# Borx25/CPU-Raytracing-experiments

Hardware: AMD Instinct MI355X
Metric: Mray/s (primary+bounce) (higher is better)
Workload: dtype f32; 1 GPU; cfg4: 4096x4096 px, S(100000) spheres + SAH BVH, MIS, Policy.max_bounces=9 (primary+8 bounces), 5 buckets, 64 accumulations/step; fixed image, tile rows split over the GPUs; image=4096x4096, spheres=100000, max_bounces=9, buckets=5, parallelism=single GPU, batches_in_flight=1, accumulations_per_batch=63, accumulations_per_batch_limit=63

## Files before the change

cpu-raytracing-experiments_amd/csrc/mirt_capi.hip:

```cpp
#include "../../include/mirt.h"
#include "kernels.hpp"
#include "bvh_layout.hpp"
#include "bvh_build.hpp"
#include "lbvh_build.hpp"

#include <hip/hip_runtime.h>
#include <algorithm>
#include <cstdarg>
#include <cstdio>
#include <cstdlib>
#include <cstring>
#include <string>
#include <vector>

using namespace mirt;

namespace {

thread_local std::string g_create_error;

struct DeviceBuffer {
	void* ptr = nullptr;
	size_t bytes = 0;
	hipError_t ensure(size_t want) {
		if (want <= bytes && ptr) return hipSuccess;
		if (ptr) { (void)hipFree(ptr); ptr = nullptr; bytes = 0; }
		if (want == 0) return hipSuccess;
		hipError_t e = hipMalloc(&ptr, want);
		if (e == hipSuccess) bytes = want;
		return e;
	}
	void release() { if (ptr) (void)hipFree(ptr); ptr = nullptr; bytes = 0; }
	template <class T> T* as() const { return static_cast<T*>(ptr); }
};

struct ScopedBuffer : DeviceBuffer {
	ScopedBuffer() = default;
	ScopedBuffer(const ScopedBuffer&) = delete;
	ScopedBuffer& operator=(const ScopedBuffer&) = delete;
	~ScopedBuffer() { release(); }
};

struct TimedLaunch { int klass; hipEvent_t start, stop; };

struct PipeSlot {
	hipStream_t stream = nullptr;
	DeviceBuffer arena;
	DeviceBuffer counts;
	DeviceBuffer contrib;
	DeviceBuffer fat;
	DeviceBuffer cand;
	hipEvent_t batch_done = nullptr;
	hipEvent_t merged = nullptr;
	hipEvent_t aov_done = nullptr;
	bool in_use = false;
	StreamBuf stream_buf[2]{};
	ShadowBuf shadow_buf{};
	HitRec* hit = nullptr;
};

}

struct mirt_ctx {
	int device = 0;
	int n_cu = 256;
	hipStream_t stream = nullptr;
	std::string error;

	mirt_policy policy{ 16, 5, 1, 0, 0, 0, 0, 0, 0, 0, 0, 0 };
	uint32_t width = 0, height = 0, h_tiles = 0, v_tiles = 0;
	uint32_t first_tile = 0, n_tiles = 0;
	uint32_t run_tiles = 0, stride_tiles = 0;
	uint32_t accumulations = 0;
	bool have_scene = false, have_camera = false;

	DeviceBuffer recs, recs_wide, spheres, prim_mat, light_sphere, light_emit, mat_albedo, mat_emission, mat_ggx, hdri;
	SceneDev scene{};
	std::vector<float> gloss_decay;
	uint32_t stream_order = 0;
	DeviceBuffer gloss_decay_dev;
	bool gloss_decay_dev_valid = false;
	CameraParams camera{};
	uint32_t bvh_depth = 0;
	bool allow_half = true;

	DeviceBuffer accumulator;
	uint32_t aov_on = 0;
	DeviceBuffer aov;
	hipEvent_t aov_prev = nullptr;
	DeviceBuffer framebuffer;
	float* frame_host = nullptr;
	size_t frame_host_bytes = 0;
	DeviceBuffer counters;
	std::vector<PipeSlot> slots;
	uint64_t planned_for = 0;
	uint32_t batch_mem_cap = 256;
	uint32_t capacity = 0;
	uint32_t seg_cap = 0;
	uint32_t arena_bounces = 0;
	uint64_t batch_seq = 0;

	uint32_t deferred = 0;
	uint32_t tune_trace_wgs = 2, tune_shade_wgs = 3, tune_chunk = kChunkMax, tune_leaf_batch = kLeafBatch, tune_refill_idle = kRefillIdle, tune_wide = 1;
	bool debug_poison_contrib = false;
	std::vector<TimedLaunch> pending;
	std::vector<hipEvent_t> free_events;
	mirt_kernel_times times{};
};

namespace {

int fail(mirt_ctx* ctx, int code, const char* fmt, ...) {
	char buf[512];
	va_list ap; va_start(ap, fmt); vsnprintf(buf, sizeof buf, fmt, ap); va_end(ap);
	if (ctx) ctx->error = buf; else g_create_error = buf;
	return code;
}
#define HIP_TRY(ctx, expr) do { hipError_t _e = (expr); if (_e != hipSuccess) return fail(ctx, MIRT_ERR_HIP, "%s: %s", #expr, hipGetErrorString(_e)); } while (0)

constexpr uint32_t kMaxBatch = 256;
constexpr uint64_t kBatchRays = 1024ull << 20;
constexpr uint64_t kSerialRays = 96ull << 20;
constexpr size_t kStreamPlanes = 2 * 10 + 2 + 14;
uint32_t pix_bits_of(const mirt_ctx* c) { uint32_t b = 8; while ((1ull << b) < static_cast<uint64_t>(c->n_tiles) * kTileSize) b++; return b; }
uint32_t max_slots(const mirt_ctx* c) {
	const uint64_t n_pix = std::max<uint64_t>(static_cast<uint64_t>(c->n_tiles) * kTileSize, 1);
	const uint64_t by_slots = ((1ull << 30) - 3ull * kSegs * kShadeBlock) / n_pix;
	return static_cast<uint32_t>(std::max<uint64_t>(std::min<uint64_t>(std::min<uint64_t>(kMaxBatch, 1u << (30u - std::min<uint32_t>(pix_bits_of(c), 24u))), by_slots), 1));
}
uint32_t batch_floor(const mirt_ctx* c) { return std::max<uint32_t>(std::min<uint32_t>(c->policy.buckets, 5u), 1u); }
uint32_t batch_limit(const mirt_ctx* c) {
	if (c->policy.max_batch) return std::min(c->policy.max_batch, max_slots(c));
	const uint64_t n_pix = static_cast<uint64_t>(c->n_tiles) * kTileSize;
	if (n_pix == 0) return 1;
	const uint64_t b = std::max<uint64_t>((kBatchRays + n_pix / 2) / n_pix, batch_floor(c));
	return static_cast<uint32_t>(std::min<uint64_t>(std::min<uint64_t>(b, max_slots(c)), std::max<uint32_t>(c->batch_mem_cap, 1u)));
// ... 6 lines not shown
	if (blocks < 1) blocks = 1;
	return static_cast<uint32_t>(blocks);
}

constexpr uint32_t kLdsPerCu = 160u * 1024u;
struct LdsPlan {
	uint32_t stack16;
	uint32_t rec_bytes, lds_recs, lds_spheres, staged_bytes, stack_bytes;
	uint32_t launch_bytes;
	uint32_t wgs_per_cu;
};
LdsPlan lds_plan(const mirt_ctx* c) {
	const SceneDev& s = c->scene;
	const bool half = s.half_boxes != 0;
	LdsPlan p{};
	p.stack16 = (half && s.n_recs <= 32768 && s.n_spheres <= 32768) ? 1u : 0u;
	p.rec_bytes = (half && !s.wide) ? 32u : 64u;
	p.stack_bytes = half ? (p.stack16 ? kLdsStack * kTraceBlock * 2u : kLdsStackWide * kTraceBlock * 4u) : kLdsStack * kTraceBlock * 4u;
	const uint32_t budget = half ? (p.stack16 ? 48u * 1024u : 32u * 1024u) : 96u * 1024u;
	if (static_cast<uint64_t>(s.n_recs) * p.rec_bytes + static_cast<uint64_t>(s.n_spheres) * 16u <= budget) { p.lds_recs = s.n_recs; p.lds_spheres = s.n_spheres; }
	else { p.lds_recs = std::min<uint32_t>(s.n_recs, budget / p.rec_bytes); p.lds_spheres = 0; }
	p.staged_bytes = p.lds_recs * p.rec_bytes + p.lds_spheres * 16u;
	p.launch_bytes = c->policy.use_bvh ? p.staged_bytes + p.stack_bytes : kBruteChunk * 16u;
	p.wgs_per_cu = std::min(std::max(kLdsPerCu / p.launch_bytes, 1u), c->tune_trace_wgs);
	return p;
}
uint32_t trace_lds(const mirt_ctx* c) { return lds_plan(c).launch_bytes; }
uint32_t trace_grid(const mirt_ctx* c, uint64_t work_items) {
	uint64_t blocks = (work_items + kTraceBlock - 1) / kTraceBlock;
	const uint64_t cap = static_cast<uint64_t>(c->n_cu) * lds_plan(c).wgs_per_cu;
	if (blocks > cap) blocks = cap;
	if (blocks < 1) blocks = 1;
	return static_cast<uint32_t>(blocks);
}

hipError_t sync_all(mirt_ctx* c) {
	for (PipeSlot& sl : c->slots) if (sl.stream) { hipError_t e = hipStreamSynchronize(sl.stream); if (e != hipSuccess) return e; }
	return hipStreamSynchronize(c->stream);
}
constexpr uint32_t kQueueWords = kSegs * kSegPitch;
constexpr uint32_t kFatCapacity = 1u << 16;
struct BatchCounters {
	uint32_t* w; uint32_t nb, seg_cap;
	static size_t words(uint32_t nb) { return static_cast<size_t>(2 * nb + 2) * kQueueWords + static_cast<size_t>(nb) * 4 + 8; }
	Queue queue(uint32_t k) const { return Queue{ w + static_cast<size_t>(k) * kQueueWords, seg_cap }; }
	uint32_t* word(uint32_t k) const { return w + static_cast<size_t>(2 * nb + 2) * kQueueWords + k; }
	Queue stream_queue(uint32_t b) const { return queue(b); }
	Queue shadow_queue(uint32_t b) const { return queue(nb + 1 + b); }
	Queue empty_queue() const { return queue(2 * nb + 1); }
	uint32_t* closest_work(uint32_t b) const { return word(b); }
	uint32_t* shadow_work(uint32_t b) const { return word(nb + b); }
	FatList fat_closest(uint32_t b, uint32_t* lists) const { return FatList{ word(2 * nb + b), lists, kFatCapacity }; }
	FatList fat_shadow(uint32_t b, uint32_t* lists) const { return FatList{ word(3 * nb + b), lists + kFatCapacity, kFatCapacity }; }
	uint32_t* cand_work() const { return word(4 * nb); }
	uint32_t* unused_fat_count() const { return word(4 * nb + 1); }
	uint32_t* listed_pixels() const { return word(4 * nb + 2); }
};
BatchCounters batch_counters(const mirt_ctx* c, const PipeSlot& sl) { return BatchCounters{ sl.counts.as<uint32_t>(), c->policy.max_bounces, c->seg_cap }; }
uint32_t wanted_slots(const mirt_ctx* c) {
	if (c->policy.streams) return std::min<uint32_t>(c->policy.streams, 8u);
	return static_cast<uint64_t>(c->n_tiles) * kTileSize * batch_limit(c) >= kSerialRays ? 1u : 3u;
}
uint64_t streams_bytes(const mirt_ctx* c) {
	const uint64_t rays = static_cast<uint64_t>(c->n_tiles) * kTileSize * batch_limit(c);
	return wanted_slots(c) * (rays * 4u * kStreamPlanes + rays * 12u);
}

void plan_batches(mirt_ctx* c) {
	const uint64_t n_pix = static_cast<uint64_t>(c->n_tiles) * kTileSize;
	if (c->policy.max_batch || n_pix == 0 || c->planned_for == n_pix) return;
	c->batch_mem_cap = kMaxBatch;
	size_t free_b = 0, total_b = 0, own = 0;
	for (const PipeSlot& sl : c->slots) own += sl.arena.bytes + sl.contrib.bytes;
	if (hipSetDevice(c->device) == hipSuccess && hipMemGetInfo(&free_b, &total_b) == hipSuccess)
		while (batch_limit(c) > batch_floor(c) && streams_bytes(c) > (free_b + own) / 5 * 4) c->batch_mem_cap = std::max(batch_limit(c) / 2, batch_floor(c));
	c->planned_for = n_pix;
}

int ensure_streams(mirt_ctx* c) {
	const uint64_t n_pix = static_cast<uint64_t>(c->n_tiles) * kTileSize;
	if (n_pix * batch_limit(c) == 0) return MIRT_OK;
	plan_batches(c);
	const uint64_t cap64 = n_pix * batch_limit(c);
	if (n_pix > (1u << 24)) return fail(c, MIRT_ERR_ARG, "more than 2^24 pixels per context (%llu); shard the tile range", (unsigned long long)n_pix);
	if (cap64 + 3ull * kSegs * kShadeBlock > (1ull << 30)) return fail(c, MIRT_ERR_ARG, "stream capacity %llu too large", (unsigned long long)cap64);
	const uint32_t seg_cap = static_cast<uint32_t>((((cap64 + kShadeBlock - 1) / kShadeBlock + kSegs - 1) / kSegs + 2) * kShadeBlock);
	const uint32_t cap = seg_cap * kSegs;
	const uint32_t nb = c->policy.max_bounces;
	const uint32_t want = wanted_slots(c);
	const size_t acc_bytes = static_cast<size_t>(c->n_tiles) * batch_limit(c) * 3 * kTileSize * sizeof(float);
	if (cap == c->capacity && nb == c->arena_bounces && c->slots.size() == want && c->slots[0].contrib.bytes >= acc_bytes) return MIRT_OK;
	HIP_TRY(c, sync_all(c));
	c->aov_prev = nullptr;
	while (c->slots.size() > want) {
		PipeSlot& sl = c->slots.back();
		sl.arena.release(); sl.counts.release(); sl.contrib.release(); sl.fat.release(); sl.cand.release();
		if (sl.batch_done) (void)hipEventDestroy(sl.batch_done);
		if (sl.merged) (void)hipEventDestroy(sl.merged);
		if (sl.aov_done) (void)hipEventDestroy(sl.aov_done);
		if (sl.stream) (void)hipStreamDestroy(sl.stream);
		c->slots.pop_back();
	}
	while (c->slots.size() < want) {
		PipeSlot sl;
		HIP_TRY(c, hipStreamCreateWithFlags(&sl.stream, hipStreamNonBlocking));
		HIP_TRY(c, hipEventCreateWithFlags(&sl.batch_done, hipEventDisableTiming));
		HIP_TRY(c, hipEventCreateWithFlags(&sl.merged, hipEventDisableTiming));
		c->slots.push_back(sl);
	}
	const size_t planes = kStreamPlanes;
	const size_t plane_bytes = (static_cast<size_t>(cap) * 4 + 255) & ~static_cast<size_t>(255);
	for (PipeSlot& sl : c->slots) {
		sl.in_use = false;
		hipError_t e = sl.arena.ensure(planes * plane_bytes);
		const char* what = "ray streams";
		if (e == hipSuccess) { e = sl.counts.ensure(BatchCounters::words(nb) * sizeof(uint32_t)); what = "queue counters"; }
		if (e == hipSuccess) { e = sl.fat.ensure(2u * kFatCapacity * sizeof(uint32_t)); what = "fat-ray lists"; }
		if (e == hipSuccess) { e = sl.cand.ensure(static_cast<size_t>(n_pix) * kCandStride * sizeof(uint32_t)); what = "candidate lists"; }
		if (e == hipSuccess) { e = sl.contrib.ensure(acc_bytes); what = "contribution buffer"; }
		if (e != hipSuccess) {
			(void)hipGetLastError();
			if (e == hipErrorOutOfMemory && !c->policy.max_batch && batch_limit(c) > batch_floor(c)) {
				for (PipeSlot& other : c->slots) { other.arena.release(); other.contrib.release(); }
				c->capacity = 0;
				c->batch_mem_cap = std::max(batch_limit(c) / 2, batch_floor(c));
				return ensure_streams(c);
			}
			return fail(c, MIRT_ERR_HIP, "%s (%zu bytes of ray streams per batch in flight): %s", what, planes * plane_bytes, hipGetErrorString(e));
		}
		char* p = sl.arena.as<char>();
		auto take = [&]() { void* r = p; p += plane_bytes; return r; };
		for (int b = 0; b < 2; b++) {
			StreamBuf& s = sl.stream_buf[b];
			s.px = (float*)take(); s.py = (float*)take(); s.pz = (float*)take();
			s.dx = (float*)take(); s.dy = (float*)take(); s.dz = (float*)take();
			s.tr = (float*)take(); s.tg = (float*)take(); s.tb = (float*)take();
			s.path = (uint32_t*)take();
		}
		sl.hit = (HitRec*)take(); (void)take();
		ShadowBuf& h = sl.shadow_buf;
		h.px = (float*)take(); h.py = (float*)take(); h.pz = (float*)take();
		h.dx = (float*)take(); h.dy = (float*)take(); h.dz = (float*)take(); h.tfar = (float*)take();
		h.sr = (float*)take(); h.sg = (float*)take(); h.sb = (float*)take();
		h.er = (float*)take(); h.eg = (float*)take(); h.eb = (float*)take();
		h.dest = (uint32_t*)take();
	}
	c->capacity = cap;
	c->seg_cap = seg_cap;
	c->arena_bounces = nb;
	return MIRT_OK;
}

size_t aov_floats(const mirt_ctx* c) { return c->aov_on ? static_cast<size_t>(c->n_tiles) * kAovPlanes * kTileSize : 0; }
int alloc_aov(mirt_ctx* c) {
	const size_t floats = aov_floats(c);
	HIP_TRY(c, c->aov.ensure(floats * sizeof(float)));
	if (floats) HIP_TRY(c, hipMemsetAsync(c->aov.ptr, 0, floats * sizeof(float), c->stream));
	return MIRT_OK;
}

int alloc_accumulator(mirt_ctx* c) {
	const size_t floats = static_cast<size_t>(c->n_tiles) * c->policy.buckets * 3 * kTileSize;
	HIP_TRY(c, sync_all(c));
	HIP_TRY(c, c->accumulator.ensure(floats * sizeof(float)));
	if (floats) HIP_TRY(c, hipMemsetAsync(c->accumulator.ptr, 0, floats * sizeof(float), c->stream));
	if (c->aov_on) { const int r = alloc_aov(c); if (r) return r; }
	HIP_TRY(c, hipMemsetAsync(c->counters.ptr, 0, sizeof(DevCounters), c->stream));
	HIP_TRY(c, hipStreamSynchronize(c->stream));
	for (PipeSlot& sl : c->slots) sl.in_use = false;
	c->accumulations = 0;
	return MIRT_OK;
// ... 47 lines not shown
	fp.inv_h_tiles = fp.h_tiles ? 1.0f / static_cast<float>(fp.h_tiles) : 0.0f;
	fp.inv_run_tiles = 1.0f / static_cast<float>(fp.run_tiles);
	return fp;
}

SceneDev trace_scene(const mirt_ctx* c) {
	SceneDev sc = c->scene;
	sc.use_bvh = c->policy.use_bvh;
	sc.chunk_max = c->tune_chunk; sc.leaf_batch = c->tune_leaf_batch; sc.refill_idle = c->tune_refill_idle;
	return sc;
}

const decltype(&k_trace<true, kPrimaryNone>) kTrace[2][3] = {
	{ k_trace<true, kPrimaryNone>, k_trace<true, kPrimaryAll>, k_trace<true, kPrimaryList> },
	{ k_trace<false, kPrimaryNone>, k_trace<false, kPrimaryAll>, k_trace<false, kPrimaryList> } };
const decltype(&k_trace_fat<true, kPrimaryNone>) kTraceFat[2][3] = {
	{ k_trace_fat<true, kPrimaryNone>, k_trace_fat<true, kPrimaryAll>, k_trace_fat<true, kPrimaryList> },
	{ k_trace_fat<false, kPrimaryNone>, k_trace_fat<false, kPrimaryAll>, k_trace_fat<false, kPrimaryList> } };
const decltype(&k_primary_cand<true>) kPrimaryCand[2] = { k_primary_cand<true>, k_primary_cand<false> };
const decltype(&k_primary_hits<true>) kPrimaryHits[2] = { k_primary_hits<true>, k_primary_hits<false> };
const decltype(&k_shade<false, false>) kShade[2][2] = { { k_shade<false, false>, k_shade<false, true> }, { k_shade<true, false>, k_shade<true, true> } };
const decltype(&k_tile_stream<false>) kTileStream[2] = { k_tile_stream<false>, k_tile_stream<true> };
static_assert(kPrimaryNone == 0 && kPrimaryAll == 1 && kPrimaryList == 2, "kTrace / kTraceFat are indexed by PRIMARY");

struct TraceLaunch {
	StreamBuf in; HitRec* hit;
	Queue closest_queue; uint32_t* closest_work;
	ShadowBuf sh; ShadowSink sink;
	Queue shadow_queue; uint32_t* shadow_work;
	FatList fat_closest, fat_shadow;
	const uint32_t* listed_pixels;
	DevCounters* ctr;
};
void launch_trace(const mirt_ctx* c, hipStream_t st, const SceneDev& sc, const FrameParams& fp, uint64_t n_rays, bool count, int primary, const TraceLaunch& t) {
	hipLaunchKernelGGL(kTrace[!count][primary], dim3(trace_grid(c, n_rays)), dim3(kTraceBlock), trace_lds(c), st, sc, fp, t.in, t.hit, t.closest_queue, t.closest_work,
	                   t.sh, t.sink, t.shadow_queue, t.shadow_work, t.fat_closest, t.fat_shadow, t.ctr);
	const uint32_t fat_grid = sc.n_spheres > 4096 ? static_cast<uint32_t>(c->n_cu) * 2u : 64u;
	if (sc.use_bvh) hipLaunchKernelGGL(kTraceFat[!count][primary], dim3(fat_grid), dim3(1024), 0, st, sc, fp, t.in, t.hit, t.fat_closest, t.sh, t.sink, t.fat_shadow, t.ctr, t.listed_pixels);
}

int launch_tile_stream(mirt_ctx* c, hipStream_t st, const SceneDev& sc, const FrameParams& fp, uint32_t batch_n, float* contrib, DevCounters* ctr, bool count) {
	if (!c->gloss_decay_dev_valid) {
		HIP_TRY(c, sync_all(c));
		HIP_TRY(c, c->gloss_decay_dev.ensure(std::max<size_t>(c->gloss_decay.size(), 1) * sizeof(float)));
		if (!c->gloss_decay.empty()) HIP_TRY(c, hipMemcpy(c->gloss_decay_dev.ptr, c->gloss_decay.data(), c->gloss_decay.size() * sizeof(float), hipMemcpyHostToDevice));
		c->gloss_decay_dev_valid = true;
	}
	Bracket t(c, MIRT_K_TRACE, st);
	hipLaunchKernelGGL(kTileStream[c->policy.brdf != 0], dim3(c->n_tiles * batch_n), dim3(kTileSize), 0, st, sc, fp, contrib, ctr, c->mat_ggx.as<float4>(),
	                   c->gloss_decay_dev.as<float>(), static_cast<uint32_t>(c->gloss_decay.size()), count ? 1u : 0u);
	return MIRT_OK;
}

int launch_first_hit_aov(mirt_ctx* c, PipeSlot& sl, hipStream_t st, const SceneDev& sc, const FrameParams& fp) {
	const bool pipelined = c->slots.size() > 1;
	if (pipelined) {
		if (!sl.aov_done) HIP_TRY(c, hipEventCreateWithFlags(&sl.aov_done, hipEventDisableTiming));
		if (c->aov_prev && c->aov_prev != sl.aov_done) HIP_TRY(c, hipStreamWaitEvent(st, c->aov_prev, 0));
	}
	{ Bracket t(c, MIRT_K_RESOLVE, st);
	  const uint32_t grid = static_cast<uint32_t>(std::min<uint64_t>((static_cast<uint64_t>(fp.n_pix) + kBlock - 1) / kBlock, static_cast<uint64_t>(c->n_cu) * 64u));
	  hipLaunchKernelGGL(k_first_hit_aov, dim3(grid), dim3(kBlock), 0, st, sc, fp, sl.hit, c->policy.brdf ? c->mat_ggx.as<float4>() : c->scene.mat_albedo, c->aov.as<float>()); }
	if (pipelined) { HIP_TRY(c, hipEventRecord(sl.aov_done, st)); c->aov_prev = sl.aov_done; }
	return MIRT_OK;
}

int launch_batch(mirt_ctx* c, uint32_t batch_n) {
	FrameParams fp = frame_params(c, c->accumulations, batch_n);
	const uint32_t nb = c->policy.max_bounces;
	const uint64_t total = static_cast<uint64_t>(fp.n_pix) * batch_n;
	if (total == 0) { c->accumulations += batch_n; return MIRT_OK; }
	const bool pipelined = c->slots.size() > 1;
	PipeSlot& sl = c->slots[c->batch_seq % c->slots.size()];
	hipStream_t st = pipelined ? sl.stream : c->stream;
	const BatchCounters bc = batch_counters(c, sl);
	const float qn = c->camera.orient[0] * c->camera.orient[0] + c->camera.orient[1] * c->camera.orient[1] + c->camera.orient[2] * c->camera.orient[2] + c->camera.orient[3] * c->camera.orient[3];
	const bool bundle = c->policy.use_bvh && c->scene.n_recs != 0 && !c->policy.trace_primary_rays && batch_n >= 3 && c->camera.z != 0.0f && std::fabs(qn - 1.0f) < 1e-4f;
	DevCounters* ctr = c->counters.as<DevCounters>();
	const float4* mat_ggx = c->mat_ggx.as<float4>();
	float* contrib = sl.contrib.as<float>();
	uint32_t* fat_lists = sl.fat.as<uint32_t>();
	const SceneDev sc = trace_scene(c);
	const bool count = c->policy.count_traffic != 0;
	const uint32_t sgrid = static_cast<uint32_t>(std::min<uint64_t>((total + kShadeBlock - 1) / kShadeBlock, static_cast<uint64_t>(c->n_cu) * c->tune_shade_wgs));
	{
		const uint64_t n_chunks = (static_cast<uint64_t>(fp.n_pix) + kShadeBlock - 1) / kShadeBlock;
		const uint64_t want = (8ull * sgrid + n_chunks - 1) / n_chunks;
		fp.first_groups = static_cast<uint32_t>(std::min<uint64_t>(std::max<uint64_t>(want, 1), batch_n));
	}

	if (pipelined && sl.in_use) HIP_TRY(c, hipStreamWaitEvent(st, sl.merged, 0));
	if (c->debug_poison_contrib)
		HIP_TRY(c, hipMemsetD32Async(reinterpret_cast<hipDeviceptr_t>(sl.contrib.ptr), 0x7fc0deadu, sl.contrib.bytes / sizeof(float), st));
	HIP_TRY(c, hipMemsetAsync(bc.w, 0, BatchCounters::words(nb) * sizeof(uint32_t), st));
	if (c->stream_order) {
		const int r = launch_tile_stream(c, st, sc, fp, batch_n, contrib, ctr, count);
		if (r) return r;
	} else {
		for (uint32_t bounce = 0; bounce < nb; bounce++) {
			const StreamBuf& in = sl.stream_buf[bounce & 1u];
			const StreamBuf& out = sl.stream_buf[(bounce & 1u) ^ 1u];
			const bool shadow_pending = fp.mis && bounce > 0;
			const bool lists = bounce == 0 && bundle;
			{ Bracket t(c, MIRT_K_TRACE, st);
			  if (lists) {
			    const FatList none{ bc.unused_fat_count(), fat_lists, 0u };
			    hipLaunchKernelGGL(kPrimaryCand[!count], dim3(trace_grid(c, fp.n_pix)), dim3(kTraceBlock), trace_lds(c), st, sc, fp, sl.cand.as<uint32_t>(), bundle_half_angle(c),
			                       bc.cand_work(), none, ctr, in.path, bc.listed_pixels());
			    const uint32_t hgrid = static_cast<uint32_t>(std::min<uint64_t>((static_cast<uint64_t>(fp.n_pix) + kBlock - 1) / kBlock, static_cast<uint64_t>(c->n_cu) * 64u));
			    hipLaunchKernelGGL(kPrimaryHits[!count], dim3(hgrid), dim3(kBlock), 0, st, sc, fp, sl.cand.as<uint32_t>(), sl.hit, ctr);
			  }
			  const ShadowSink sink{ in.path, in.px, in.py, in.pz, contrib, batch_n, fp.pix_bits, nullptr };
			  const TraceLaunch tl{ in, sl.hit, lists ? Queue{ bc.listed_pixels(), 0u } : bc.stream_queue(bounce), bc.closest_work(bounce),
			                        sl.shadow_buf, sink, shadow_pending ? bc.shadow_queue(bounce - 1) : bc.empty_queue(), bc.shadow_work(shadow_pending ? bounce - 1 : 0),
			                        bc.fat_closest(bounce, fat_lists), bc.fat_shadow(bounce, fat_lists), bc.listed_pixels(), ctr };
			  launch_trace(c, st, sc, fp, total, count, lists ? kPrimaryList : bounce == 0 ? kPrimaryAll : kPrimaryNone, tl); }
			if (bounce == 0 && c->aov_on) { const int r = launch_first_hit_aov(c, sl, st, sc, fp); if (r) return r; }
			{ Bracket t(c, MIRT_K_SHADE, st);
			  const float decay = bounce < c->gloss_decay.size() ? c->gloss_decay[bounce] : 0.0f;
			  hipLaunchKernelGGL(kShade[bounce == 0][c->policy.brdf != 0], dim3(sgrid), dim3(kShadeBlock), 0, st, sc, fp, in, sl.hit, out, sl.shadow_buf, bounce,
			                     bc.stream_queue(bounce), bc.stream_queue(bounce + 1), bc.shadow_queue(bounce), contrib, ctr, mat_ggx, decay); }
		}
	}
	HIP_TRY(c, hipGetLastError());
	if (pipelined) {
		HIP_TRY(c, hipEventRecord(sl.batch_done, st));
		HIP_TRY(c, hipStreamWaitEvent(c->stream, sl.batch_done, 0));
	}
	{ Bracket t(c, MIRT_K_RESOLVE);
	  hipLaunchKernelGGL(k_merge_contrib, dim3(grid_for(c, static_cast<uint64_t>(c->n_tiles) * (kTileSize / 4u))), dim3(kBlock), 0, c->stream,
	                     c->accumulator.as<float4>(), sl.contrib.as<float4>(), c->n_tiles, c->policy.buckets, batch_n, fp.acc_base); }
	HIP_TRY(c, hipGetLastError());
	if (pipelined) { HIP_TRY(c, hipEventRecord(sl.merged, c->stream)); sl.in_use = true; }
	c->batch_seq++;
	c->accumulations += batch_n;
	if (c->policy.profile && c->pending.size() > 512) harvest(c);
	return MIRT_OK;
}

template <class T>
int upload(mirt_ctx* c, DeviceBuffer& buf, const std::vector<T>& host) {
	HIP_TRY(c, buf.ensure(std::max<size_t>(host.size(), 1) * sizeof(T)));
	if (!host.empty()) HIP_TRY(c, hipMemcpyAsync(buf.ptr, host.data(), host.size() * sizeof(T), hipMemcpyHostToDevice, c->stream));
	return MIRT_OK;
}

int check_ready(mirt_ctx* c) {
	if (!c) return MIRT_ERR_ARG;
	if (!c->have_scene) return fail(c, MIRT_ERR_STATE, "mirt_set_scene has not been called");
	if (!c->have_camera) return fail(c, MIRT_ERR_STATE, "mirt_set_camera has not been called");
	if (c->width == 0 && c->height == 0) return fail(c, MIRT_ERR_STATE, "mirt_resize has not been called");
	return MIRT_OK;
}

int flush_deferred(mirt_ctx* c) {
	if (!c->deferred) return MIRT_OK;
	const uint32_t n = c->deferred;
	c->deferred = 0;
	HIP_TRY(c, hipSetDevice(c->device));
	int r = ensure_streams(c); if (r) return r;
	return launch_batch(c, n);
}

struct SceneArgs {
	const mirt_sphere *geometry, *bvh_prims; uint32_t n_spheres;
	const mirt_bvh_node* nodes; uint32_t n_nodes;
	const mirt_material* materials; uint32_t n_materials;
	const int32_t* lights; uint32_t n_lights;
// ... 156 lines not shown
	tl.closest_queue = bc.stream_queue(0); tl.closest_work = bc.closest_work(0);
	tl.shadow_queue = bc.shadow_queue(0); tl.shadow_work = bc.shadow_work(0);
	tl.fat_closest = bc.fat_closest(0, fat.as<uint32_t>()); tl.fat_shadow = bc.fat_shadow(0, fat.as<uint32_t>());
	tl.ctr = ctr.as<DevCounters>();
	{ Bracket t(c, MIRT_K_TRACE);
	  launch_trace(c, c->stream, trace_scene(c), FrameParams{}, n, false, kPrimaryNone, tl); }
	hipError_t e = hipGetLastError();
	if (e == hipSuccess) e = hipStreamSynchronize(c->stream);
	if (e == hipSuccess) e = hipMemcpy(result, res.ptr, result_bytes, hipMemcpyDeviceToHost);
	if (e != hipSuccess) return fail(c, MIRT_ERR_HIP, "%s: %s", who, hipGetErrorString(e));
	return MIRT_OK;
}

}

extern "C" {

const char* mirt_last_error(const mirt_ctx* ctx) { return ctx ? ctx->error.c_str() : g_create_error.c_str(); }

int mirt_create(int device, mirt_ctx** out) {
	if (!out) return fail(nullptr, MIRT_ERR_ARG, "out is NULL");
	*out = nullptr;
	int n = 0;
	hipError_t e = hipGetDeviceCount(&n);
	if (e != hipSuccess || n <= 0) return fail(nullptr, MIRT_ERR_NO_DEVICE, "no HIP device available (%s); mirt has no CPU path", hipGetErrorString(e));
	if (device < 0 || device >= n) return fail(nullptr, MIRT_ERR_ARG, "device %d out of range (have %d)", device, n);
	e = hipSetDevice(device);
	if (e != hipSuccess) return fail(nullptr, MIRT_ERR_HIP, "hipSetDevice: %s", hipGetErrorString(e));
	mirt_ctx* c = new mirt_ctx();
	c->device = device;
	if (const char* e = std::getenv("MIRT_TUNE_CHUNK")) c->tune_chunk = static_cast<uint32_t>(std::min(std::max(std::atoi(e), 64), 65536)) & ~63u;
	if (const char* e = std::getenv("MIRT_TUNE_REFILL_IDLE")) c->tune_refill_idle = static_cast<uint32_t>(std::min(std::max(std::atoi(e), 1), 64));
	if (const char* e = std::getenv("MIRT_TUNE_WIDE")) c->tune_wide = std::atoi(e) != 0 ? 1u : 0u;
	if (const char* e = std::getenv("MIRT_TUNE_LEAF_BATCH")) c->tune_leaf_batch = static_cast<uint32_t>(std::min(std::max(std::atoi(e), 1), 64));
	if (const char* e = std::getenv("MIRT_TUNE_TRACE_WGS")) c->tune_trace_wgs = std::atoi(e) == 1 ? 1u : 2u;
	if (const char* e = std::getenv("MIRT_TUNE_SHADE_WGS")) c->tune_shade_wgs = static_cast<uint32_t>(std::min(std::max(std::atoi(e), 1), 16));
	if (const char* e = std::getenv("MIRT_DEBUG_POISON_CONTRIB")) c->debug_poison_contrib = std::atoi(e) != 0;
	hipDeviceProp_t prop;
	if (hipGetDeviceProperties(&prop, device) == hipSuccess) c->n_cu = prop.multiProcessorCount > 0 ? prop.multiProcessorCount : 256;
	e = hipStreamCreateWithFlags(&c->stream, hipStreamNonBlocking);
	if (e == hipSuccess) e = c->counters.ensure(sizeof(DevCounters));
	if (e == hipSuccess) e = hipMemsetAsync(c->counters.ptr, 0, sizeof(DevCounters), c->stream);
	if (e != hipSuccess) { int r = fail(nullptr, MIRT_ERR_HIP, "context setup: %s", hipGetErrorString(e)); delete c; return r; }
	*out = c;
	return MIRT_OK;
}

int mirt_destroy(mirt_ctx* c) {
	if (!c) return MIRT_ERR_ARG;
	(void)hipSetDevice(c->device);
	(void)sync_all(c);
	harvest(c);
	for (PipeSlot& sl : c->slots) {
		sl.arena.release(); sl.counts.release(); sl.contrib.release(); sl.fat.release(); sl.cand.release();
		if (sl.batch_done) (void)hipEventDestroy(sl.batch_done);
		if (sl.merged) (void)hipEventDestroy(sl.merged);
		if (sl.aov_done) (void)hipEventDestroy(sl.aov_done);
		if (sl.stream) (void)hipStreamDestroy(sl.stream);
	}
	c->slots.clear();
	for (hipEvent_t e : c->free_events) (void)hipEventDestroy(e);
	DeviceBuffer* bufs[] = { &c->recs, &c->recs_wide, &c->spheres, &c->prim_mat, &c->light_sphere, &c->light_emit, &c->mat_albedo, &c->mat_emission,
	                         &c->mat_ggx, &c->hdri, &c->accumulator, &c->aov, &c->framebuffer, &c->counters, &c->gloss_decay_dev };
	for (DeviceBuffer* b : bufs) b->release();
	if (c->frame_host) (void)hipHostFree(c->frame_host);
	if (c->stream) (void)hipStreamDestroy(c->stream);
	delete c;
	return MIRT_OK;
}

int mirt_set_scene(mirt_ctx* c, const mirt_sphere* geometry, const mirt_sphere* bvh_prims, uint32_t n_spheres,
                   const mirt_bvh_node* nodes, uint32_t n_nodes, const mirt_material* materials, uint32_t n_materials,
                   const int32_t* lights, uint32_t n_lights, const float ambient_color[3],
                   const float* hdri_rgba, uint32_t hdri_w, uint32_t hdri_h) {
	if (!c) return MIRT_ERR_ARG;
	{ const int fr = flush_deferred(c); if (fr) return fr; }
	const SceneArgs a{ geometry, bvh_prims, n_spheres, nodes, n_nodes, materials, n_materials, lights, n_lights, ambient_color, hdri_rgba, hdri_w, hdri_h };
	int r = check_scene_args(c, a); if (r) return r;
	HIP_TRY(c, hipSetDevice(c->device));
	const SceneTables t = flatten_tables(a);
	SceneRecords tree;
	if ((r = upload(c, c->spheres, t.sph)) || (r = build_scene_records(c, a, t.sph, tree)) || (r = upload(c, c->prim_mat, t.pm)) ||
	    (r = upload(c, c->light_sphere, t.lsp)) || (r = upload(c, c->light_emit, t.lem)) || (r = upload(c, c->mat_albedo, t.alb)) ||
	    (r = upload(c, c->mat_emission, t.emi)) || (r = upload(c, c->mat_ggx, t.ggx)) || (r = upload(c, c->hdri, t.sky))) return r;
	HIP_TRY(c, hipStreamSynchronize(c->stream));
	commit_scene(c, a, tree);
	if ((r = plan_trace_lds(c))) return r;
	c->have_scene = true;
	return MIRT_OK;
}

int mirt_set_camera(mirt_ctx* c, const float pos[3], const float orient_xyzw[4], float half_width, float half_height, float z, float exposure) {
	if (!c) return MIRT_ERR_ARG;
	if (!pos || !orient_xyzw) return fail(c, MIRT_ERR_ARG, "pos / orient is NULL");
	if (c->have_camera && std::memcmp(c->camera.pos, pos, 12) == 0 && std::memcmp(c->camera.orient, orient_xyzw, 16) == 0 &&
	    c->camera.half_width == half_width && c->camera.half_height == half_height && c->camera.z == z && c->camera.exposure == exposure)
		return MIRT_OK;
	{ const int fr = flush_deferred(c); if (fr) return fr; }
	for (int k = 0; k < 3; k++) c->camera.pos[k] = pos[k];
	for (int k = 0; k < 4; k++) c->camera.orient[k] = orient_xyzw[k];
	c->camera.half_width = half_width; c->camera.half_height = half_height; c->camera.z = z; c->camera.exposure = exposure;
	c->have_camera = true;
	return MIRT_OK;
}

int mirt_set_policy(mirt_ctx* c, const mirt_policy* p) {
	if (!c || !p) return MIRT_ERR_ARG;
	if (p->max_bounces < 1 || p->max_bounces > 1024) return fail(c, MIRT_ERR_ARG, "max_bounces %u out of range", p->max_bounces);
	if (p->buckets < 1 || p->buckets > MIRT_MAX_BUCKETS) return fail(c, MIRT_ERR_ARG, "buckets %u out of range 1..%u", p->buckets, MIRT_MAX_BUCKETS);
	if (p->brdf > 1) return fail(c, MIRT_ERR_ARG, "brdf %u is neither 0 (Lambertian) nor 1 (GGX)", p->brdf);
	{ const int fr = flush_deferred(c); if (fr) return fr; }
	HIP_TRY(c, hipSetDevice(c->device));
	HIP_TRY(c, sync_all(c));
	const bool realloc_acc = p->buckets != c->policy.buckets;
	const bool replan = p->max_batch != c->policy.max_batch || p->streams != c->policy.streams || p->buckets != c->policy.buckets || p->max_bounces != c->policy.max_bounces;
	c->policy = *p;
	if (replan) c->planned_for = 0;
	if (realloc_acc && c->n_tiles) { int r = alloc_accumulator(c); if (r) return r; }
	return MIRT_OK;
}
int mirt_set_gloss_decay(mirt_ctx* c, const float* decay, uint32_t n) {
	if (!c) return MIRT_ERR_ARG;
	if (!decay) n = 0;
	if (n > 1024) return fail(c, MIRT_ERR_ARG, "gloss decay table of %u entries (at most 1024, the max_bounces limit)", n);
	for (uint32_t i = 0; i < n; i++)
		if (!(decay[i] >= 0.0f && decay[i] <= 1.0f)) return fail(c, MIRT_ERR_ARG, "gloss decay[%u] = %g is not in [0, 1]", i, static_cast<double>(decay[i]));
	{ const int fr = flush_deferred(c); if (fr) return fr; }
	c->gloss_decay.assign(decay, decay + n);
	c->gloss_decay_dev_valid = false;
	return MIRT_OK;
}
int mirt_set_stream_order(mirt_ctx* c, uint32_t exact) {
	if (!c) return MIRT_ERR_ARG;
	if (exact > 1) return fail(c, MIRT_ERR_ARG, "stream order %u is neither 0 (any order, FMA form for every ray) nor 1 (the reference's slots and scalar tail)", exact);
	if (exact == c->stream_order) return MIRT_OK;
	if (exact && c->aov_on) return fail(c, MIRT_ERR_STATE, "exact stream order keeps no hit records (k_tile_stream runs a tile's whole bounce loop in one launch), so it cannot feed the first-hit AOVs: call mirt_set_aov(ctx, 0) first");
	{ const int fr = flush_deferred(c); if (fr) return fr; }
	c->stream_order = exact;
	return MIRT_OK;
}
int mirt_get_stream_order(const mirt_ctx* c, uint32_t* exact) { if (!c || !exact) return MIRT_ERR_ARG; *exact = c->stream_order; return MIRT_OK; }
int mirt_get_policy(const mirt_ctx* c, mirt_policy* p) {
	if (!c || !p) return MIRT_ERR_ARG;
	*p = c->policy;
	plan_batches(const_cast<mirt_ctx*>(c));
	p->max_batch = batch_limit(c);
	p->streams = wanted_slots(c);
	return MIRT_OK;
}

int mirt_resize(mirt_ctx* c, uint32_t width, uint32_t height) {
	if (!c) return MIRT_ERR_ARG;
	if (width > 65536 || height > 65536) return fail(c, MIRT_ERR_ARG, "size %ux%u too large", width, height);
	c->deferred = 0;
	HIP_TRY(c, hipSetDevice(c->device));
	HIP_TRY(c, sync_all(c));
	c->width = width; c->height = height;
	c->h_tiles = width / MIRT_TILE_ROOT; c->v_tiles = height / MIRT_TILE_ROOT;
	c->first_tile = 0; c->n_tiles = c->h_tiles * c->v_tiles; c->run_tiles = 0; c->stride_tiles = 0;
	HIP_TRY(c, c->framebuffer.ensure(std::max<size_t>(static_cast<size_t>(width) * height, 1) * sizeof(float4)));
	HIP_TRY(c, hipMemsetAsync(c->framebuffer.ptr, 0, c->framebuffer.bytes, c->stream));
	if (c->frame_host_bytes < c->framebuffer.bytes) {
		if (c->frame_host) (void)hipHostFree(c->frame_host);
		c->frame_host = nullptr; c->frame_host_bytes = 0;
		HIP_TRY(c, hipHostMalloc(reinterpret_cast<void**>(&c->frame_host), c->framebuffer.bytes, hipHostMallocDefault));
		c->frame_host_bytes = c->framebuffer.bytes;
	}
	return alloc_accumulator(c);
}

int mirt_set_tile_range(mirt_ctx* c, uint32_t first_tile, uint32_t n_tiles) {
	if (!c) return MIRT_ERR_ARG;
	const uint64_t all = static_cast<uint64_t>(c->h_tiles) * c->v_tiles;
	if (static_cast<uint64_t>(first_tile) + n_tiles > all) return fail(c, MIRT_ERR_ARG, "tile range [%u,+%u) exceeds %llu tiles", first_tile, n_tiles, (unsigned long long)all);
	c->deferred = 0;
	HIP_TRY(c, hipSetDevice(c->device));
	HIP_TRY(c, sync_all(c));
	c->first_tile = first_tile; c->n_tiles = n_tiles; c->run_tiles = 0; c->stride_tiles = 0;
	return alloc_accumulator(c);
}

int mirt_set_tile_rows(mirt_ctx* c, uint32_t first_row, uint32_t row_stride) {
	if (!c) return MIRT_ERR_ARG;
	if (row_stride == 0) return fail(c, MIRT_ERR_ARG, "row_stride must be at least 1");
	c->deferred = 0;
	HIP_TRY(c, hipSetDevice(c->device));
	HIP_TRY(c, sync_all(c));
	const uint32_t rows = first_row < c->v_tiles ? (c->v_tiles - first_row + row_stride - 1) / row_stride : 0u;
	c->first_tile = first_row * c->h_tiles; c->n_tiles = rows * c->h_tiles;
	c->run_tiles = c->h_tiles; c->stride_tiles = row_stride > 1 ? row_stride * c->h_tiles : 0u;
	return alloc_accumulator(c);
}

int mirt_reset(mirt_ctx* c) {
	if (!c) return MIRT_ERR_ARG;
	c->deferred = 0;
	HIP_TRY(c, hipSetDevice(c->device));
	return alloc_accumulator(c);
}

int mirt_accumulate_async(mirt_ctx* c, uint32_t n_calls) {
	int r = check_ready(c); if (r) return r;
	HIP_TRY(c, hipSetDevice(c->device));
	if ((r = ensure_streams(c))) return r;
	if (c->n_tiles == 0) { c->accumulations += n_calls; return MIRT_OK; }
	const uint32_t limit = batch_limit(c);
	uint64_t total = static_cast<uint64_t>(c->deferred) + n_calls;
	c->deferred = 0;
	while (total >= limit) {
		if ((r = launch_batch(c, limit))) return r;
		total -= limit;
	}
	c->deferred = static_cast<uint32_t>(total);
	return MIRT_OK;
}
int mirt_synchronize(mirt_ctx* c) {
	if (!c) return MIRT_ERR_ARG;
	{ const int fr = flush_deferred(c); if (fr) return fr; }
	HIP_TRY(c, hipSetDevice(c->device));
	HIP_TRY(c, sync_all(c));
	return MIRT_OK;
}
int mirt_accumulate(mirt_ctx* c, uint32_t n_calls) {
	int r = mirt_accumulate_async(c, n_calls);
	if (r) return r;
	return mirt_synchronize(c);
}
int mirt_get_accumulations(const mirt_ctx* c, uint32_t* a) { if (!c || !a) return MIRT_ERR_ARG; *a = c->accumulations + c->deferred; return MIRT_OK; }

int mirt_accumulator_floats(const mirt_ctx* c, size_t* n) {
	if (!c || !n) return MIRT_ERR_ARG;
	*n = static_cast<size_t>(c->n_tiles) * c->policy.buckets * 3 * kTileSize;
	return MIRT_OK;
}
int mirt_read_accumulator(mirt_ctx* c, float* dst) {
	if (!c || !dst) return MIRT_ERR_ARG;
	size_t n = 0; mirt_accumulator_floats(c, &n);
	{ const int fr = flush_deferred(c); if (fr) return fr; }
	HIP_TRY(c, hipSetDevice(c->device));
	HIP_TRY(c, sync_all(c));
	if (n) HIP_TRY(c, hipMemcpy(dst, c->accumulator.ptr, n * sizeof(float), hipMemcpyDeviceToHost));
	return MIRT_OK;
}
// ... 169 lines not shown
	const StreamBuf& s = c->slots[0].stream_buf[0];
	float* srcs[6] = { s.px, s.py, s.pz, s.dx, s.dy, s.dz };
	for (int k = 0; k < 3; k++) {
		HIP_TRY(c, hipMemcpy(p_xyz + k * n, srcs[k], n * 4, hipMemcpyDeviceToHost));
		HIP_TRY(c, hipMemcpy(dir_xyz + k * n, srcs[3 + k], n * 4, hipMemcpyDeviceToHost));
	}
	return MIRT_OK;
}

int mirt_debug_trace_closest(mirt_ctx* c, size_t n, const float* p_xyz, const float* dir_xyz, float* tfar_out, int32_t* prim_out) {
	if (!c) return MIRT_ERR_ARG;
	if (!c->have_scene) return fail(c, MIRT_ERR_STATE, "mirt_set_scene has not been called");
	if (!p_xyz || !dir_xyz || !tfar_out || !prim_out || n == 0 || n >= (1ull << 31)) return fail(c, MIRT_ERR_ARG, "bad arguments");
	std::vector<HitRec> hits(n);
	const int r = debug_trace(c, "debug_trace_closest", n, p_xyz, dir_xyz, nullptr, hits.data());
	if (r == MIRT_OK) for (size_t i = 0; i < n; i++) { tfar_out[i] = hits[i].tfar; prim_out[i] = hits[i].prim; }
	return r;
}

int mirt_debug_trace_shadow(mirt_ctx* c, size_t n, const float* p_xyz, const float* dir_xyz, const float* tfar, uint8_t* occluded_out) {
	if (!c) return MIRT_ERR_ARG;
	if (!c->have_scene) return fail(c, MIRT_ERR_STATE, "mirt_set_scene has not been called");
	if (!p_xyz || !dir_xyz || !tfar || !occluded_out || n == 0 || n >= (1ull << 31)) return fail(c, MIRT_ERR_ARG, "bad arguments");
	std::vector<uint32_t> occ(n);
	const int r = debug_trace(c, "debug_trace_shadow", n, p_xyz, dir_xyz, tfar, occ.data());
	if (r == MIRT_OK) for (size_t i = 0; i < n; i++) occluded_out[i] = occ[i] ? 1 : 0;
	return r;
}

int mirt_debug_math(mirt_ctx* c, int fn, size_t n, const float* in, float* out) {
	if (!c) return MIRT_ERR_ARG;
	static const int n_in[11] = { 1, 2, 1, 2, 2, 6, 8, 3, 10, 9, 1 }, n_out[11] = { 2, 1, 1, 3, 3, 10, 5, 5, 3, 6, 1 };
	if (fn < 0 || fn > 10 || !in || !out || n == 0 || n >= (1u << 28)) return fail(c, MIRT_ERR_ARG, "bad arguments");
	HIP_TRY(c, hipSetDevice(c->device));
	ScopedBuffer din, dout;
	HIP_TRY(c, din.ensure(n * n_in[fn] * 4)); HIP_TRY(c, dout.ensure(n * n_out[fn] * 4));
	HIP_TRY(c, hipMemcpy(din.ptr, in, n * n_in[fn] * 4, hipMemcpyHostToDevice));
	hipLaunchKernelGGL(k_debug_math, dim3(grid_for(c, n)), dim3(kBlock), 0, c->stream, fn, static_cast<uint32_t>(n), din.as<float>(), dout.as<float>());
	hipError_t e = hipGetLastError();
	if (e == hipSuccess) e = hipStreamSynchronize(c->stream);
	if (e == hipSuccess) e = hipMemcpy(out, dout.ptr, n * n_out[fn] * 4, hipMemcpyDeviceToHost);
	if (e != hipSuccess) return fail(c, MIRT_ERR_HIP, "debug_math: %s", hipGetErrorString(e));
	return MIRT_OK;
}

int mirt_debug_primary_lists(mirt_ctx* c, uint32_t hist[10]) {
	int r = check_ready(c); if (r) return r;
	if (!hist) return fail(c, MIRT_ERR_ARG, "hist is NULL");
	if (!c->policy.use_bvh || c->scene.n_recs == 0 || c->n_tiles == 0) return fail(c, MIRT_ERR_STATE, "needs policy.use_bvh, a tree and at least one tile");
	{ const int fr = flush_deferred(c); if (fr) return fr; }
	HIP_TRY(c, hipSetDevice(c->device));
	if ((r = ensure_streams(c))) return r;
	HIP_TRY(c, sync_all(c));
	PipeSlot& sl = c->slots[0];
	const FrameParams fp = frame_params(c, 0, 1);
	SceneDev sc = trace_scene(c);
	sc.use_bvh = 1;
	const BatchCounters bc = batch_counters(c, sl);
	HIP_TRY(c, hipMemsetAsync(bc.w, 0, BatchCounters::words(bc.nb) * sizeof(uint32_t), c->stream));
	const FatList none{ bc.unused_fat_count(), sl.fat.as<uint32_t>(), 0u };
	const bool count = false;
	hipLaunchKernelGGL(kPrimaryCand[!count], dim3(trace_grid(c, fp.n_pix)), dim3(kTraceBlock), trace_lds(c), c->stream, sc, fp, sl.cand.as<uint32_t>(), bundle_half_angle(c),
	                   bc.cand_work(), none, c->counters.as<DevCounters>(), static_cast<uint32_t*>(nullptr), bc.listed_pixels());
	HIP_TRY(c, hipGetLastError());
	std::vector<uint32_t> host(static_cast<size_t>(fp.n_pix));
	HIP_TRY(c, hipMemcpyAsync(host.data(), sl.cand.ptr, host.size() * 4, hipMemcpyDeviceToHost, c->stream));
	HIP_TRY(c, hipStreamSynchronize(c->stream));
	for (int k = 0; k < 10; k++) hist[k] = 0;
	for (size_t p = 0; p < fp.n_pix; p++) { const uint32_t n = host[p]; hist[n == kCandOverflow ? 9 : std::min<uint32_t>(n, 8u)]++; }
	return MIRT_OK;
}

int mirt_debug_info(mirt_ctx* c, uint32_t out[8]) {
	if (!c || !out) return MIRT_ERR_ARG;
	const SceneDev& s = c->scene;
	const LdsPlan p = lds_plan(c);
	out[0] = s.n_recs; out[1] = s.lds_recs; out[2] = s.lds_spheres; out[3] = c->bvh_depth; out[4] = s.half_boxes | (s.wide << 1);
	out[5] = p.launch_bytes; out[6] = p.wgs_per_cu; out[7] = static_cast<uint32_t>(c->n_cu);
	return MIRT_OK;
}
int mirt_debug_allow_half_boxes(mirt_ctx* c, int allow) { if (!c) return MIRT_ERR_ARG; c->allow_half = allow != 0; return MIRT_OK; }

}
```

Measured before the change: 9304 Mray/s.

## Cache primary-ray candidate lists across batches until camera or scene changes

Moves the per-pixel primary candidate lists from each pipeline slot into the context. The candidate-building kernel now runs once and is reused by later batches, with an event that pipelined slots wait on. The lists are invalidated when the camera, scene, tile range, resolution or relevant policy fields change. This removes a full-image candidate trace from every batch, at the cost of extra invalidation bookkeeping and a separate listed-pixel buffer. Bundling is also disabled in stream-order mode.

```diff
diff --git a/cpu-raytracing-experiments_amd/csrc/mirt_capi.hip b/cpu-raytracing-experiments_amd/csrc/mirt_capi.hip
--- a/cpu-raytracing-experiments_amd/csrc/mirt_capi.hip
+++ b/cpu-raytracing-experiments_amd/csrc/mirt_capi.hip
@@ -49,11 +49,11 @@
 	DeviceBuffer counts;
 	DeviceBuffer contrib;
 	DeviceBuffer fat;
-	DeviceBuffer cand;
 	hipEvent_t batch_done = nullptr;
 	hipEvent_t merged = nullptr;
 	hipEvent_t aov_done = nullptr;
 	bool in_use = false;
+	uint64_t cand_gen = 0;
 	StreamBuf stream_buf[2]{};
 	ShadowBuf shadow_buf{};
 	HitRec* hit = nullptr;
@@ -82,6 +82,12 @@
 	bool gloss_decay_dev_valid = false;
 	CameraParams camera{};
 	uint32_t bvh_depth = 0;
+	DeviceBuffer cand;
+	DeviceBuffer cand_listed;
+	DeviceBuffer cand_words;
+	hipEvent_t cand_built = nullptr;
+	uint64_t cand_gen = 0;
+	bool cand_valid = false;
 	bool allow_half = true;
 
 	DeviceBuffer accumulator;
@@ -194,9 +200,13 @@
 	uint32_t* shadow_work(uint32_t b) const { return word(nb + b); }
 	FatList fat_closest(uint32_t b, uint32_t* lists) const { return FatList{ word(2 * nb + b), lists, kFatCapacity }; }
 	FatList fat_shadow(uint32_t b, uint32_t* lists) const { return FatList{ word(3 * nb + b), lists + kFatCapacity, kFatCapacity }; }
-	uint32_t* cand_work() const { return word(4 * nb); }
-	uint32_t* unused_fat_count() const { return word(4 * nb + 1); }
-	uint32_t* listed_pixels() const { return word(4 * nb + 2); }
+};
+struct CandWords {
+	uint32_t* w;
+	static constexpr size_t kWords = 4;
+	uint32_t* work() const { return w; }
+	uint32_t* unused_fat_count() const { return w + 1; }
+	uint32_t* listed_pixels() const { return w + 2; }
 };
 BatchCounters batch_counters(const mirt_ctx* c, const PipeSlot& sl) { return BatchCounters{ sl.counts.as<uint32_t>(), c->policy.max_bounces, c->seg_cap }; }
 uint32_t wanted_slots(const mirt_ctx* c) {
@@ -236,7 +246,7 @@
 	c->aov_prev = nullptr;
 	while (c->slots.size() > want) {
 		PipeSlot& sl = c->slots.back();
-		sl.arena.release(); sl.counts.release(); sl.contrib.release(); sl.fat.release(); sl.cand.release();
+		sl.arena.release(); sl.counts.release(); sl.contrib.release(); sl.fat.release();
 		if (sl.batch_done) (void)hipEventDestroy(sl.batch_done);
 		if (sl.merged) (void)hipEventDestroy(sl.merged);
 		if (sl.aov_done) (void)hipEventDestroy(sl.aov_done);
@@ -258,7 +268,6 @@
 		const char* what = "ray streams";
 		if (e == hipSuccess) { e = sl.counts.ensure(BatchCounters::words(nb) * sizeof(uint32_t)); what = "queue counters"; }
 		if (e == hipSuccess) { e = sl.fat.ensure(2u * kFatCapacity * sizeof(uint32_t)); what = "fat-ray lists"; }
-		if (e == hipSuccess) { e = sl.cand.ensure(static_cast<size_t>(n_pix) * kCandStride * sizeof(uint32_t)); what = "candidate lists"; }
 		if (e == hipSuccess) { e = sl.contrib.ensure(acc_bytes); what = "contribution buffer"; }
 		if (e != hipSuccess) {
 			(void)hipGetLastError();
@@ -412,6 +421,24 @@
 	return MIRT_OK;
 }
 
+int build_primary_lists(mirt_ctx* c, const SceneDev& sc, const FrameParams& fp, bool count) {
+	HIP_TRY(c, c->cand.ensure(static_cast<size_t>(fp.n_pix) * kCandStride * sizeof(uint32_t)));
+	HIP_TRY(c, c->cand_listed.ensure(static_cast<size_t>(fp.n_pix) * sizeof(uint32_t)));
+	HIP_TRY(c, c->cand_words.ensure(CandWords::kWords * sizeof(uint32_t)));
+	if (!c->cand_built) HIP_TRY(c, hipEventCreateWithFlags(&c->cand_built, hipEventDisableTiming));
+	const CandWords cw{ c->cand_words.as<uint32_t>() };
+	HIP_TRY(c, hipMemsetAsync(cw.w, 0, CandWords::kWords * sizeof(uint32_t), c->stream));
+	{ Bracket t(c, MIRT_K_TRACE);
+	  const FatList none{ cw.unused_fat_count(), nullptr, 0u };
+	  hipLaunchKernelGGL(kPrimaryCand[!count], dim3(trace_grid(c, fp.n_pix)), dim3(kTraceBlock), trace_lds(c), c->stream, sc, fp, c->cand.as<uint32_t>(), bundle_half_angle(c),
+	                     cw.work(), none, c->counters.as<DevCounters>(), c->cand_listed.as<uint32_t>(), cw.listed_pixels()); }
+	HIP_TRY(c, hipGetLastError());
+	HIP_TRY(c, hipEventRecord(c->cand_built, c->stream));
+	c->cand_gen++;
+	c->cand_valid = true;
+	return MIRT_OK;
+}
+
 int launch_first_hit_aov(mirt_ctx* c, PipeSlot& sl, hipStream_t st, const SceneDev& sc, const FrameParams& fp) {
 	const bool pipelined = c->slots.size() > 1;
 	if (pipelined) {
@@ -435,7 +462,7 @@
 	hipStream_t st = pipelined ? sl.stream : c->stream;
 	const BatchCounters bc = batch_counters(c, sl);
 	const float qn = c->camera.orient[0] * c->camera.orient[0] + c->camera.orient[1] * c->camera.orient[1] + c->camera.orient[2] * c->camera.orient[2] + c->camera.orient[3] * c->camera.orient[3];
-	const bool bundle = c->policy.use_bvh && c->scene.n_recs != 0 && !c->policy.trace_primary_rays && batch_n >= 3 && c->camera.z != 0.0f && std::fabs(qn - 1.0f) < 1e-4f;
+	const bool bundle = c->policy.use_bvh && c->scene.n_recs != 0 && !c->policy.trace_primary_rays && batch_n >= 3 && c->camera.z != 0.0f && std::fabs(qn - 1.0f) < 1e-4f && !c->stream_order;
 	DevCounters* ctr = c->counters.as<DevCounters>();
 	const float4* mat_ggx = c->mat_ggx.as<float4>();
 	float* contrib = sl.contrib.as<float>();
@@ -453,6 +480,11 @@
 	if (c->debug_poison_contrib)
 		HIP_TRY(c, hipMemsetD32Async(reinterpret_cast<hipDeviceptr_t>(sl.contrib.ptr), 0x7fc0deadu, sl.contrib.bytes / sizeof(float), st));
 	HIP_TRY(c, hipMemsetAsync(bc.w, 0, BatchCounters::words(nb) * sizeof(uint32_t), st));
+	if (bundle) {
+		if (!c->cand_valid || count) { const int r = build_primary_lists(c, sc, fp, count); if (r) return r; }
+		if (pipelined && sl.cand_gen != c->cand_gen) { HIP_TRY(c, hipStreamWaitEvent(st, c->cand_built, 0)); sl.cand_gen = c->cand_gen; }
+	}
+	const CandWords cw{ c->cand_words.as<uint32_t>() };
 	if (c->stream_order) {
 		const int r = launch_tile_stream(c, st, sc, fp, batch_n, contrib, ctr, count);
 		if (r) return r;
@@ -464,16 +496,15 @@
 			const bool lists = bounce == 0 && bundle;
 			{ Bracket t(c, MIRT_K_TRACE, st);
 			  if (lists) {
-			    const FatList none{ bc.unused_fat_count(), fat_lists, 0u };
-			    hipLaunchKernelGGL(kPrimaryCand[!count], dim3(trace_grid(c, fp.n_pix)), dim3(kTraceBlock), trace_lds(c), st, sc, fp, sl.cand.as<uint32_t>(), bundle_half_angle(c),
-			                       bc.cand_work(), none, ctr, in.path, bc.listed_pixels());
 			    const uint32_t hgrid = static_cast<uint32_t>(std::min<uint64_t>((static_cast<uint64_t>(fp.n_pix) + kBlock - 1) / kBlock, static_cast<uint64_t>(c->n_cu) * 64u));
-			    hipLaunchKernelGGL(kPrimaryHits[!count], dim3(hgrid), dim3(kBlock), 0, st, sc, fp, sl.cand.as<uint32_t>(), sl.hit, ctr);
+			    hipLaunchKernelGGL(kPrimaryHits[!count], dim3(hgrid), dim3(kBlock), 0, st, sc, fp, c->cand.as<uint32_t>(), sl.hit, ctr);
 			  }
 			  const ShadowSink sink{ in.path, in.px, in.py, in.pz, contrib, batch_n, fp.pix_bits, nullptr };
-			  const TraceLaunch tl{ in, sl.hit, lists ? Queue{ bc.listed_pixels(), 0u } : bc.stream_queue(bounce), bc.closest_work(bounce),
+			  StreamBuf rays = in;
+			  if (lists) rays.path = c->cand_listed.as<uint32_t>();
+			  const TraceLaunch tl{ rays, sl.hit, lists ? Queue{ cw.listed_pixels(), 0u } : bc.stream_queue(bounce), bc.closest_work(bounce),
 			                        sl.shadow_buf, sink, shadow_pending ? bc.shadow_queue(bounce - 1) : bc.empty_queue(), bc.shadow_work(shadow_pending ? bounce - 1 : 0),
-			                        bc.fat_closest(bounce, fat_lists), bc.fat_shadow(bounce, fat_lists), bc.listed_pixels(), ctr };
+			                        bc.fat_closest(bounce, fat_lists), bc.fat_shadow(bounce, fat_lists), lists ? cw.listed_pixels() : nullptr, ctr };
 			  launch_trace(c, st, sc, fp, total, count, lists ? kPrimaryList : bounce == 0 ? kPrimaryAll : kPrimaryNone, tl); }
 			if (bounce == 0 && c->aov_on) { const int r = launch_first_hit_aov(c, sl, st, sc, fp); if (r) return r; }
 			{ Bracket t(c, MIRT_K_SHADE, st);
@@ -736,7 +767,7 @@
 	(void)sync_all(c);
 	harvest(c);
 	for (PipeSlot& sl : c->slots) {
-		sl.arena.release(); sl.counts.release(); sl.contrib.release(); sl.fat.release(); sl.cand.release();
+		sl.arena.release(); sl.counts.release(); sl.contrib.release(); sl.fat.release();
 		if (sl.batch_done) (void)hipEventDestroy(sl.batch_done);
 		if (sl.merged) (void)hipEventDestroy(sl.merged);
 		if (sl.aov_done) (void)hipEventDestroy(sl.aov_done);
@@ -745,9 +776,11 @@
 	c->slots.clear();
 	for (hipEvent_t e : c->free_events) (void)hipEventDestroy(e);
 	DeviceBuffer* bufs[] = { &c->recs, &c->recs_wide, &c->spheres, &c->prim_mat, &c->light_sphere, &c->light_emit, &c->mat_albedo, &c->mat_emission,
-	                         &c->mat_ggx, &c->hdri, &c->accumulator, &c->aov, &c->framebuffer, &c->counters, &c->gloss_decay_dev };
+	                         &c->mat_ggx, &c->hdri, &c->accumulator, &c->aov, &c->framebuffer, &c->counters, &c->gloss_decay_dev,
+	                         &c->cand, &c->cand_listed, &c->cand_words };
 	for (DeviceBuffer* b : bufs) b->release();
 	if (c->frame_host) (void)hipHostFree(c->frame_host);
+	if (c->cand_built) (void)hipEventDestroy(c->cand_built);
 	if (c->stream) (void)hipStreamDestroy(c->stream);
 	delete c;
 	return MIRT_OK;
@@ -768,6 +801,7 @@
 	    (r = upload(c, c->light_sphere, t.lsp)) || (r = upload(c, c->light_emit, t.lem)) || (r = upload(c, c->mat_albedo, t.alb)) ||
 	    (r = upload(c, c->mat_emission, t.emi)) || (r = upload(c, c->mat_ggx, t.ggx)) || (r = upload(c, c->hdri, t.sky))) return r;
 	HIP_TRY(c, hipStreamSynchronize(c->stream));
+	c->cand_valid = false;
 	commit_scene(c, a, tree);
 	if ((r = plan_trace_lds(c))) return r;
 	c->have_scene = true;
@@ -785,6 +819,7 @@
 	for (int k = 0; k < 4; k++) c->camera.orient[k] = orient_xyzw[k];
 	c->camera.half_width = half_width; c->camera.half_height = half_height; c->camera.z = z; c->camera.exposure = exposure;
 	c->have_camera = true;
+	c->cand_valid = false;
 	return MIRT_OK;
 }
 
@@ -798,6 +833,8 @@
 	HIP_TRY(c, sync_all(c));
 	const bool realloc_acc = p->buckets != c->policy.buckets;
 	const bool replan = p->max_batch != c->policy.max_batch || p->streams != c->policy.streams || p->buckets != c->policy.buckets || p->max_bounces != c->policy.max_bounces;
+	if (p->use_bvh != c->policy.use_bvh || p->gpu_build != c->policy.gpu_build || p->reference_tree != c->policy.reference_tree || p->trace_primary_rays != c->policy.trace_primary_rays)
+		c->cand_valid = false;
 	c->policy = *p;
 	if (replan) c->planned_for = 0;
 	if (realloc_acc && c->n_tiles) { int r = alloc_accumulator(c); if (r) return r; }
@@ -840,6 +877,7 @@
 	HIP_TRY(c, hipSetDevice(c->device));
 	HIP_TRY(c, sync_all(c));
 	c->width = width; c->height = height;
+	c->cand_valid = false;
 	c->h_tiles = width / MIRT_TILE_ROOT; c->v_tiles = height / MIRT_TILE_ROOT;
 	c->first_tile = 0; c->n_tiles = c->h_tiles * c->v_tiles; c->run_tiles = 0; c->stride_tiles = 0;
 	HIP_TRY(c, c->framebuffer.ensure(std::max<size_t>(static_cast<size_t>(width) * height, 1) * sizeof(float4)));
@@ -861,6 +899,7 @@
 	HIP_TRY(c, hipSetDevice(c->device));
 	HIP_TRY(c, sync_all(c));
 	c->first_tile = first_tile; c->n_tiles = n_tiles; c->run_tiles = 0; c->stride_tiles = 0;
+	c->cand_valid = false;
 	return alloc_accumulator(c);
 }
 
@@ -873,6 +912,7 @@
 	const uint32_t rows = first_row < c->v_tiles ? (c->v_tiles - first_row + row_stride - 1) / row_stride : 0u;
 	c->first_tile = first_row * c->h_tiles; c->n_tiles = rows * c->h_tiles;
 	c->run_tiles = c->h_tiles; c->stride_tiles = row_stride > 1 ? row_stride * c->h_tiles : 0u;
+	c->cand_valid = false;
 	return alloc_accumulator(c);
 }
 
@@ -1148,19 +1188,10 @@
 	HIP_TRY(c, hipSetDevice(c->device));
 	if ((r = ensure_streams(c))) return r;
 	HIP_TRY(c, sync_all(c));
-	PipeSlot& sl = c->slots[0];
 	const FrameParams fp = frame_params(c, 0, 1);
-	SceneDev sc = trace_scene(c);
-	sc.use_bvh = 1;
-	const BatchCounters bc = batch_counters(c, sl);
-	HIP_TRY(c, hipMemsetAsync(bc.w, 0, BatchCounters::words(bc.nb) * sizeof(uint32_t), c->stream));
-	const FatList none{ bc.unused_fat_count(), sl.fat.as<uint32_t>(), 0u };
-	const bool count = false;
-	hipLaunchKernelGGL(kPrimaryCand[!count], dim3(trace_grid(c, fp.n_pix)), dim3(kTraceBlock), trace_lds(c), c->stream, sc, fp, sl.cand.as<uint32_t>(), bundle_half_angle(c),
-	                   bc.cand_work(), none, c->counters.as<DevCounters>(), static_cast<uint32_t*>(nullptr), bc.listed_pixels());
-	HIP_TRY(c, hipGetLastError());
+	if (!c->cand_valid && (r = build_primary_lists(c, trace_scene(c), fp, false))) return r;
 	std::vector<uint32_t> host(static_cast<size_t>(fp.n_pix));
-	HIP_TRY(c, hipMemcpyAsync(host.data(), sl.cand.ptr, host.size() * 4, hipMemcpyDeviceToHost, c->stream));
+	HIP_TRY(c, hipMemcpyAsync(host.data(), c->cand.ptr, host.size() * 4, hipMemcpyDeviceToHost, c->stream));
 	HIP_TRY(c, hipStreamSynchronize(c->stream));
 	for (int k = 0; k < 10; k++) hist[k] = 0;
 	for (size_t p = 0; p < fp.n_pix; p++) { const uint32_t n = host[p]; hist[n == kCandOverflow ? 9 : std::min<uint32_t>(n, 8u)]++; }
```

After: 9422 Mray/s (median of 6 runs). 1.01x the previous value.
